# vbronetskyi/nclt-slam-project

Hardware: AMD Instinct MI355X
Metric: relocalization frames/sec @640x480, 10k-landmark DB; Hamming-match HBM GB/s (higher is better)
Workload: dtype u8; 1 GPU; 640x480 BGR frames, 10000-record landmark DB (640000 descriptors, rows=fixed64), global relocalization tick per frame: ORB(500) + whole-DB mutual Hamming scan + top-25 PnP-RANSAC(200); frames resident in HBM, every frame's 96-byte result record written to pinned host memory by the tick's last kernel; distinct_frames=32, preroll_steps=20, streams=4, records=10000, descriptors=640000, parallelism=frames sharded across ranks, database replicated, no collective

## Files before the change

### nclt-slam-project_amd/csrc/reloc_orb.hip

```cpp
#include <math.h>

#include "../../include/reloc_orb_pattern.h"
#include "reloc_internal.h"
#include "reloc_pixels.h"

static_assert(HARRIS_CHUNK == 1024, "k_harris reads one dword per thread");

__constant__ signed char c_pattern[RELOC_ORB_NTESTS * 4];
__constant__ int c_umax[16] = {15, 15, 15, 15, 14, 14, 14, 13, 13, 12, 11, 10, 9, 8, 6, 3};
__constant__ signed char c_ring_dx[16] = {0, 1, 2, 3, 3, 3, 2, 1, 0, -1, -2, -3, -3, -3, -2, -1};
__constant__ signed char c_ring_dy[16] = {3, 3, 2, 1, 0, -1, -2, -3, -3, -3, -2, -1, 0, 1, 2, 3};

__device__ __forceinline__ int find_level(const int *base, int id)
{
    int l = 0;
#pragma unroll
    for (int k = 1; k < NLEV; ++k) l += id >= base[k];
    return l;
}


struct OrbBatch { OrbFrame f[RELOC_BATCH_MAX]; };

__device__ __forceinline__ void pyr_tab_index(const OrbTable *__restrict__ tab, const PyrTile &T, const int (&tbase)[NLEV + 1], int i,
// ... 248 lines not shown
        const int v = (int)p[c_ring_dy[k] * stride + c_ring_dx[k]] - c;
        bright |= (u32)(v > thr) << k;
        dark |= (u32)(v < -thr) << k;
    }
    auto run9 = [](u32 m) {
        u32 x = m | (m << 16);
        u32 y = x & (x >> 1);
        y &= y >> 2;
        y &= y >> 4;
        y &= x >> 8;
        return (y & 0xFFFFu) != 0;
    };
    return run9(bright) ? 1 : (run9(dark) ? -1 : 0);
}

__device__ int fast_corner_score(const uint8_t *p, int stride, int thr, int sign)
{
    const int c = p[0];
    int v[16];
#pragma unroll
    for (int k = 0; k < 16; ++k) v[k] = sign * ((int)p[c_ring_dy[k] * stride + c_ring_dx[k]] - c);
    int m2[16], m4[16], best = 0;
#pragma unroll
    for (int k = 0; k < 16; ++k) m2[k] = min(v[k], v[(k + 1) & 15]);
#pragma unroll
    for (int k = 0; k < 16; ++k) m4[k] = min(m2[k], m2[(k + 2) & 15]);
#pragma unroll
    for (int k = 0; k < 16; ++k) {
        const int m8 = min(m4[k], m4[(k + 4) & 15]);
        const int m9 = min(m8, v[(k + 8) & 15]);
        best = max(best, m9);
    }
    return best > thr ? best - 1 : 0;
}

__device__ __forceinline__ bool fast_run9(u32 x)
{
    u32 y = x & (x >> 1);
    y &= y >> 2;
    y &= y >> 4;
    y &= x >> 8;
    return (y & 0xFFFFu) != 0;
}

struct FastQuad {
    u32 nb[2], nd[2];
    const u32 (*w)[3];
    __device__ __forceinline__ FastQuad(const u32 (&rows)[7][3], int thr) : w(rows)
    {
        const u32 c = rows[3][1];
        const u32 ce = c & 0x00FF00FFu, co = (c >> 8) & 0x00FF00FFu;
        const u32 t2 = (0x7FFFu - (u32)thr) * 0x00010001u;
        nb[0] = t2 - ce; nb[1] = t2 - co;
        nd[0] = t2 + ce; nd[1] = t2 + co;
    }
    template <int DX, int DY>
    __device__ __forceinline__ void flags(u32 (&tb)[2], u32 (&td)[2]) const
    {
        constexpr int b = 4 + DX, q = b >> 2, o = b & 3;
        constexpr u32 sel_e = (u32)o | 0x0C00u | (u32)(o + 2) << 16 | 0x0C000000u;
        constexpr u32 sel_o = (u32)(o + 1) | 0x0C00u | (u32)(o + 3) << 16 | 0x0C000000u;
        const u32 ve = __builtin_amdgcn_perm(w[DY + 3][q + 1], w[DY + 3][q], sel_e);
        const u32 vo = __builtin_amdgcn_perm(w[DY + 3][q + 1], w[DY + 3][q], sel_o);
        tb[0] = ve + nb[0]; tb[1] = vo + nb[1];
        td[0] = nd[0] - ve; td[1] = nd[1] - vo;
    }
    template <int K>
    __device__ __forceinline__ void ring(u32 (&tb)[2], u32 (&td)[2]) const
    {
        constexpr int dx[16] = {0, 1, 2, 3, 3, 3, 2, 1, 0, -1, -2, -3, -3, -3, -2, -1};
        constexpr int dy[16] = {3, 3, 2, 1, 0, -1, -2, -3, -3, -3, -2, -1, 0, 1, 2, 3};
        flags<dx[K], dy[K]>(tb, td);
    }
    __device__ __forceinline__ bool candidate() const
    {
        u32 b0[2], d0[2], b4[2], d4[2], b8[2], d8[2], b12[2], d12[2];
        ring<0>(b0, d0); ring<4>(b4, d4); ring<8>(b8, d8); ring<12>(b12, d12);
        u32 any = 0;
#pragma unroll
        for (int j = 0; j < 2; ++j) {
            any |= (b0[j] & b4[j]) | (b8[j] & b12[j]) | ((b0[j] | b4[j]) & (b8[j] | b12[j]));
            any |= (d0[j] & d4[j]) | (d8[j] & d12[j]) | ((d0[j] | d4[j]) & (d8[j] | d12[j]));
        }
        return (any & 0x80008000u) != 0;
    }
    template <int K>
    __device__ __forceinline__ void shift_in(u32 (&mb)[2], u32 (&md)[2]) const
    {
        u32 tb[2], td[2];
        ring<K>(tb, td);
#pragma unroll
        for (int j = 0; j < 2; ++j) {
            mb[j] = (tb[j] & 0x80008000u) | ((mb[j] >> 1) & 0x7FFF7FFFu);
            md[j] = (td[j] & 0x80008000u) | ((md[j] >> 1) & 0x7FFF7FFFu);
        }
        if constexpr (K < 15) shift_in<K + 1>(mb, md);
    }
    __device__ __forceinline__ void masks(u32 (&mb)[2], u32 (&md)[2]) const
    {
        mb[0] = mb[1] = md[0] = md[1] = 0;
        shift_in<0>(mb, md);
    }
};

constexpr int FT_P = FT / 4 + 3;
static_assert(FT == 32, "fast_nms_tile maps 256 lanes to 32 rows x 8 dwords");
template <bool MASKED, int THR>
__device__ __forceinline__ void fast_nms_tile(const OrbTable *__restrict__ tab, const uint8_t *__restrict__ pyr,
                                              uint8_t *__restrict__ nms, int32_t *__restrict__ hist, int bid,
                                              const uint8_t *__restrict__ mask)
{
    __shared__ u32 s_img4[(FT + 8) * FT_P];
    __shared__ u32 s_sc4[(FT + 2) * (FT + 4) / 4];
    __shared__ unsigned short s_corner[(FT + 2) * (FT + 2)];
    __shared__ int s_nc;
    __shared__ int s_hist[256];
    const uint8_t *const s_img = reinterpret_cast<const uint8_t *>(s_img4);
    uint8_t *const s_sc = reinterpret_cast<uint8_t *>(s_sc4);
    const int l = find_level(tab->fast_tile_base, bid);
    const OrbLevel L = tab->lev[l];
    const int tile = bid - tab->fast_tile_base[l];
    const int tx = L.stride / FT;
    const int x0 = (tile % tx) * FT, y0 = (tile / tx) * FT;
    const int tid = threadIdx.x;
    const int e = RELOC_ORB_EDGE;
    const int thr = THR ? THR : tab->fast_thr;
    uint8_t *out = nms + L.off;
    const bool live = L.quota > 0 && x0 + FT > e && x0 < L.w - e && y0 + FT > e && y0 < L.h - e;
    if (!live) {
        const int y = y0 + tid / 8, x = x0 + (tid % 8) * 4;
        if (y < L.h) *reinterpret_cast<u32 *>(out + (size_t)y * L.stride + x) = 0;
        return;
    }
    s_hist[tid] = 0;
    const uint8_t *src = pyr + L.off;
    const int IS = 4 * FT_P;
    {
        const int r16 = tid >> 4, c16 = tid & 15;
        u32 v[3];
#pragma unroll
        for (int t = 0; t < 3; ++t) {
            const int ry = 16 * t + r16;
            if (c16 < FT / 4 + 2 && ry < FT + 8) {
                const int gy = min(max(y0 + ry - 4, 0), L.h - 1);
                v[t] = halo_dword<false>(src + (size_t)gy * L.stride, x0 - 4 + 4 * c16, L.w);
            }
        }
#pragma unroll
        for (int t = 0; t < 3; ++t) {
            const int ry = 16 * t + r16;
            if (c16 < FT / 4 + 2 && ry < FT + 8) s_img4[ry * FT_P + c16] = v[t];
        }
    }
    for (int i = tid; i < (FT + 2) * (FT + 4) / 4; i += 256) s_sc4[i] = 0;
    if (tid == 0) s_nc = 0;
    __syncthreads();
    const int SS = FT + 4;
    {
        const int ry = 1 + (tid >> 3), g = tid & 7, rx = 1 + 4 * g;
        u32 w[7][3];
#pragma unroll
        for (int r = 0; r < 7; ++r)
#pragma unroll
            for (int q = 0; q < 3; ++q) w[r][q] = s_img4[(ry + r) * FT_P + g + q];
        const FastQuad Q(w, thr);
        if (__any(Q.candidate())) {
            u32 mb[2], md[2];
            Q.masks(mb, md);
            const int gy = y0 + ry - 1;
            const bool row_in = gy >= 3 && gy < L.h - 3;
#pragma unroll
            for (int k = 0; k < 4; ++k) {
                const u32 sel = (k & 2) ? 0x03020302u : 0x01000100u;
                const bool br = fast_run9(__builtin_amdgcn_perm(mb[k & 1], mb[k & 1], sel));
                const bool dk = fast_run9(__builtin_amdgcn_perm(md[k & 1], md[k & 1], sel));
                const int gx = x0 + rx - 1 + k;
                if ((br || dk) && row_in && gx >= 3 && gx < L.w - 3)
                    s_corner[atomicAdd(&s_nc, 1)] = (unsigned short)((ry << 6) | (rx + k) | (br ? 0 : 0x8000));
            }
        }
    }
    {
        const int i = tid;
        const int ry = i < FT + 2 ? 0 : (i < 2 * (FT + 2) ? FT + 1 : (i < 3 * FT + 4 ? i - (2 * FT + 3) : i - (3 * FT + 3)));
        const int rx = i < FT + 2 ? i : (i < 2 * (FT + 2) ? i - (FT + 2) : (i < 3 * FT + 4 ? 0 : FT + 1));
        const int gy = y0 + ry - 1, gx = x0 + rx - 1;
        int pol = 0;
        bool cand = false;
        const uint8_t *pc = s_img + (ry + 3) * IS + (rx + 3);
        const bool inside = i < 4 * FT + 4 && gx >= 3 && gx < L.w - 3 && gy >= 3 && gy < L.h - 3;
        if (inside) {
            const int c = pc[0];
            const int v0 = (int)pc[3 * IS] - c, v4 = (int)pc[3] - c, v8 = (int)pc[-3 * IS] - c, v12 = (int)pc[-3] - c;
            const int nb = (v0 > thr) + (v4 > thr) + (v8 > thr) + (v12 > thr);
            const int nd = (v0 < -thr) + (v4 < -thr) + (v8 < -thr) + (v12 < -thr);
            cand = nb >= 2 || nd >= 2;
        }
        if (tid < 3 * 64 && __any(cand)) {
            if (cand) pol = fast_is_corner(pc, IS, thr);
        }
        if (pol) s_corner[atomicAdd(&s_nc, 1)] = (unsigned short)((ry << 6) | rx | (pol < 0 ? 0x8000 : 0));
    }
    __syncthreads();
    for (int i = tid; i < s_nc; i += 256) {
        const int e16 = s_corner[i], ry = (e16 >> 6) & 63, rx = e16 & 63;
        s_sc[ry * SS + rx] = (uint8_t)fast_corner_score(s_img + (ry + 3) * IS + (rx + 3), IS, thr, (e16 & 0x8000) ? -1 : 1);
    }
    __syncthreads();
    {
        const int ry = tid / 8, rx4 = (tid % 8) * 4;
        u32 word = 0;
        u32 keep = 0;
        if constexpr (MASKED)
            if (y0 + ry < L.h) keep = *reinterpret_cast<const u32 *>(mask + L.off + (size_t)(y0 + ry) * L.stride + x0 + rx4);
#pragma unroll
        for (int k = 0; k < 4; ++k) {
            const int gx = x0 + rx4 + k, gy = y0 + ry;
            const uint8_t *s = s_sc + (ry + 1) * SS + (rx4 + k + 1);
            const int c = (!MASKED || ((keep >> (8 * k)) & 0xFF)) ? s[0] : 0;
            if (c && gx >= e && gx < L.w - e && gy >= e && gy < L.h - e && c > s[-1] && c > s[1] && c > s[-SS - 1] &&
                c > s[-SS] && c > s[-SS + 1] && c > s[SS - 1] && c > s[SS] && c > s[SS + 1]) {
                word |= (u32)c << (8 * k);
                atomicAdd(&s_hist[c], 1);
            }
        }
        const int gy = y0 + ry;
        if (gy < L.h) *reinterpret_cast<u32 *>(out + (size_t)gy * L.stride + x0 + rx4) = word;
    }
    __syncthreads();
    if (s_hist[tid]) atomicAdd(&hist[l * 256 + tid], s_hist[tid]);
}

template <bool MASKED, int THR>
__global__ __launch_bounds__(256) void k_fast_blur(const OrbTable *__restrict__ tab, const uint8_t *__restrict__ pyr,
                                                   uint8_t *__restrict__ nms, int32_t *__restrict__ hist,
                                                   uint8_t *__restrict__ blur, int n_fast, const uint8_t *__restrict__ mask)
{
    RELOC_SMALL_KERNEL_PRIO();
    if ((int)blockIdx.x < n_fast) fast_nms_tile<MASKED, THR>(tab, pyr, nms, hist, (int)blockIdx.x, mask);
    else blur7_tile(tab, pyr, blur, (int)blockIdx.x - n_fast);
}
template <bool MASKED, int THR>
__global__ __launch_bounds__(256) void k_fast_blur_batch(OrbBatch b, int n_fast)
{
    RELOC_SMALL_KERNEL_PRIO();
    const OrbFrame &F = b.f[blockIdx.y];
    if ((int)blockIdx.x < n_fast) fast_nms_tile<MASKED, THR>(F.tab, F.pyr, F.nms, F.hist, (int)blockIdx.x, F.mask);
    else blur7_tile(F.tab, F.pyr, F.blur, (int)blockIdx.x - n_fast);
}

__global__ __launch_bounds__(256) void k_mask_level(const OrbTable *__restrict__ tab, const int32_t *__restrict__ rz,
                                                    uint8_t *__restrict__ mp, int l)
{
    const OrbLevel S = tab->lev[l - 1], D = tab->lev[l];
    const int x4 = 4 * (int)(blockIdx.x * 256 + threadIdx.x), y = (int)blockIdx.y;
    if (x4 >= D.stride || y >= D.h) return;
    const int32_t *xo = rz + tab->rz_off[l][0], *xc = rz + tab->rz_off[l][1];
    const int sy0 = rz[tab->rz_off[l][2] + y], sy1 = sy0 + 1 < S.h ? sy0 + 1 : S.h - 1;
    const u32 b = (u32)rz[tab->rz_off[l][3] + y], one = 1u << RELOC_RESIZE_COEF_BITS;
    const uint8_t *r0 = mp + S.off + (size_t)sy0 * S.stride, *r1 = mp + S.off + (size_t)sy1 * S.stride;
    u32 out = 0;
#pragma unroll
    for (int k = 0; k < 4; ++k) {
        if (x4 + k < D.w) {
            const int k0 = xo[x4 + k], k1 = k0 + 1 < S.w ? k0 + 1 : S.w - 1;
            const u32 a = (u32)xc[x4 + k];
            const u32 h0 = (u32)r0[k0] * (one - a) + (u32)r0[k1] * a;
            const u32 h1 = (u32)r1[k0] * (one - a) + (u32)r1[k1] * a;
            const u32 v = (h0 * (one - b) + h1 * b + (1u << 15)) >> 16;
            if (v > RELOC_ORB_MASK_THRESH) out |= v << (8 * k);
        }
    }
    *reinterpret_cast<u32 *>(mp + D.off + (size_t)y * D.stride + x4) = out;
}

__device__ int stage1_cut_wave(const int32_t *__restrict__ hist_l, int n_keep, int lane, int thr)
{
    const int4 h = *reinterpret_cast<const int4 *>(hist_l + 4 * lane);
    const int mine = h.x + h.y + h.z + h.w;
    int incl = mine;
#pragma unroll
    for (int d = 1; d < 64; d <<= 1) {
        const int v = __shfl_down(incl, d);
        if (lane + d < 64) incl += v;
    }
    const int above = incl - mine;
    const int c3 = h.w + above, c2 = h.z + c3, c1 = h.y + c2, c0 = h.x + c1;
    const int total = __builtin_amdgcn_readlane(c0, 0);
    int cut0 = thr;
    if (total > n_keep) {
        const int s = c3 >= n_keep ? 3 : (c2 >= n_keep ? 2 : (c1 >= n_keep ? 1 : (c0 >= n_keep ? 0 : -1)));
        cut0 = (int)wave_max_u32(s < 0 ? 0u : (unsigned)(4 * lane + s + 1)) - 1;
    }
    unsigned best = 0;
    const int cs[4] = {c0, c1, c2, c3};
#pragma unroll
    for (int k = 3; k >= 0; --k) {
        const int s = 4 * lane + k;
        if (s >= cut0 && (cs[k] <= RELOC_ORB_STAGE1_CAP || s == 255)) best = (unsigned)(256 - s);
    }
    return 256 - (int)wave_max_u32(best);
}

__device__ __forceinline__ void harris_terms(const uint8_t *p, int step, int lane, int &a, int &b, int &c)
{
    a = b = c = 0;
    if (lane < 49) {
        const int dy = lane / 7 - 3, dx = lane % 7 - 3;
        const uint8_t *q = p + dy * step + dx;
        const int ix = (q[1] - q[-1]) * 2 + (q[-step + 1] - q[-step - 1]) + (q[step + 1] - q[step - 1]);
        const int iy = (q[step] - q[-step]) * 2 + (q[step - 1] - q[-step - 1]) + (q[step + 1] - q[-step + 1]);
        a = ix * ix; b = iy * iy; c = ix * iy;
    }
}

__device__ __forceinline__ float harris_finish(int a, int b, int c)
{
    a = wave_sum_i32(a);
    b = wave_sum_i32(b);
    c = wave_sum_i32(c);
    const float scale = __fdiv_rn(1.f, (float)((1 << 2) * RELOC_HARRIS_BLOCK) * 255.f);
    const float s2 = __fmul_rn(scale, scale), s3 = __fmul_rn(s2, scale), s4 = __fmul_rn(s3, scale);
    const float fa = (float)a, fb = (float)b, fc = (float)c;
    const float t1 = __fmul_rn(fa, fb), t2 = __fmul_rn(fc, fc), t3 = __fadd_rn(fa, fb);
    const float t4 = __fmul_rn(RELOC_HARRIS_K, t3), t5 = __fmul_rn(t4, t3);
    const float t6 = __fsub_rn(t1, t2), t7 = __fsub_rn(t6, t5);
    return __fmul_rn(t7, s4);
}

enum { ORB_MODE_DEFAULT = 0, ORB_MODE_HARRIS = 1, ORB_MODE_FAST = 2 };
template <int MODE>
__device__ __forceinline__ void harris_body(const OrbTable *__restrict__ tab, const uint8_t *__restrict__ pyr,
                                                const uint8_t *__restrict__ nms, const int32_t *__restrict__ hist,
                                                int32_t *__restrict__ cand_cnt, u32 *__restrict__ cand_key,
                                                float *__restrict__ cand_resp, int32_t *__restrict__ dbg_cut)
{
    __shared__ int s_cut;
    __shared__ int s_n, s_base;
    __shared__ u32 s_list[HARRIS_CHUNK];
    const int thr = MODE == ORB_MODE_DEFAULT ? RELOC_FAST_THRESHOLD : tab->fast_thr;
    const int l = find_level(tab->flat_base, blockIdx.x);
    const OrbLevel L = tab->lev[l];
    if (L.quota <= 0 || L.w <= 2 * RELOC_ORB_EDGE || L.h <= 2 * RELOC_ORB_EDGE) return;
    const int64_t idx0 = ((int64_t)(blockIdx.x - tab->flat_base[l]) * 256 + threadIdx.x) * (HARRIS_CHUNK / 256);
    const int64_t total = (int64_t)L.stride * L.h;
    u32 v = 0;
    if (idx0 < total) v = *reinterpret_cast<const u32 *>(nms + L.off + idx0);
    const bool any = v != 0;
    if (threadIdx.x == 0) s_n = 0;
    if (!__syncthreads_or(any)) return;
    if (threadIdx.x < 64) {
        const int c = stage1_cut_wave(hist + l * 256, MODE == ORB_MODE_FAST ? L.quota : 2 * L.quota, threadIdx.x, thr);
        if (threadIdx.x == 0) {
            s_cut = c;
            if (dbg_cut) dbg_cut[l] = c;
        }
    }
    __syncthreads();
    const int cut = s_cut;
    if constexpr (MODE == ORB_MODE_FAST) {
        if (any) {
#pragma unroll
            for (int k = 0; k < HARRIS_CHUNK / 256; ++k) {
                const int sc = (v >> (8 * k)) & 0xFF;
                if (sc && sc >= cut) {
                    const int64_t idx = idx0 + k;
                    const int y = (int)(idx / L.stride), x = (int)(idx % L.stride);
                    const int pos = atomicAdd(&cand_cnt[l], 1);
                    if (pos < RELOC_ORB_STAGE1_CAP) {
                        cand_key[(size_t)l * RELOC_ORB_STAGE1_CAP + pos] = ((u32)y << 16) | (u32)x;
                        cand_resp[(size_t)l * RELOC_ORB_STAGE1_CAP + pos] = (float)sc;
                    }
                }
            }
        }
        return;
    }
    if (any) {
#pragma unroll
        for (int k = 0; k < HARRIS_CHUNK / 256; ++k) {
            const int sc = (v >> (8 * k)) & 0xFF;
            if (sc && sc >= cut) {
                const int64_t idx = idx0 + k;
                const int y = (int)(idx / L.stride), x = (int)(idx % L.stride);
                s_list[atomicAdd(&s_n, 1)] = ((u32)y << 16) | (u32)x;
            }
        }
    }
    __syncthreads();
    const int n = s_n;
    const int lane = threadIdx.x & 63, wave = threadIdx.x >> 6;
    const uint8_t *img = pyr + L.off;
    int base_ret = 0;
    if (threadIdx.x == 0 && n > 0) base_ret = atomicAdd(&cand_cnt[l], n);
    auto terms = [&](u32 key, int &a, int &b, int &c) {
        harris_terms(img + (size_t)(key >> 16) * L.stride + (key & 0xFFFF), L.stride, lane, a, b, c);
    };
    int i = wave * 2;
    const bool first = i < n;
    u32 k0 = 0, k1 = 0;
    int a0 = 0, b0 = 0, c0 = 0, a1 = 0, b1 = 0, c1 = 0;
    float h0 = 0.f, h1 = 0.f;
    if (first) {
        k0 = s_list[i]; k1 = s_list[i + 1 < n ? i + 1 : i];
        terms(k0, a0, b0, c0);
        terms(k1, a1, b1, c1);
    }
    if (threadIdx.x == 0) s_base = base_ret;
    if (first) { h0 = harris_finish(a0, b0, c0); h1 = harris_finish(a1, b1, c1); }
    __syncthreads();
    const int base = s_base;
    auto put = [&](int at, u32 key, float r) {
        const int pos = base + at;
        if (pos < RELOC_ORB_STAGE1_CAP) {
            cand_key[(size_t)l * RELOC_ORB_STAGE1_CAP + pos] = key;
            cand_resp[(size_t)l * RELOC_ORB_STAGE1_CAP + pos] = r;
        }
    };
    if (first && lane == 0) {
        put(i, k0, h0);
        if (i + 1 < n) put(i + 1, k1, h1);
    }
    for (i += 8; i < n; i += 8) {
        k0 = s_list[i]; k1 = s_list[i + 1 < n ? i + 1 : i];
        terms(k0, a0, b0, c0);
        terms(k1, a1, b1, c1);
        h0 = harris_finish(a0, b0, c0);
        h1 = harris_finish(a1, b1, c1);
        if (lane == 0) {
            put(i, k0, h0);
            if (i + 1 < n) put(i + 1, k1, h1);
        }
    }
}
template <int MODE>
__global__ __launch_bounds__(256) void k_harris(const OrbTable *__restrict__ tab, const uint8_t *__restrict__ pyr,
                                                const uint8_t *__restrict__ nms, const int32_t *__restrict__ hist,
                                                int32_t *__restrict__ cand_cnt, u32 *__restrict__ cand_key,
                                                float *__restrict__ cand_resp, int32_t *__restrict__ dbg_cut)
{
    RELOC_SMALL_KERNEL_PRIO();
    harris_body<MODE>(tab, pyr, nms, hist, cand_cnt, cand_key, cand_resp, dbg_cut);
}
template <int MODE>
__global__ __launch_bounds__(256) void k_harris_batch(OrbBatch b)
{
    RELOC_SMALL_KERNEL_PRIO();
    const OrbFrame &F = b.f[blockIdx.y];
    harris_body<MODE>(F.tab, F.pyr, F.nms, F.hist, F.cand_cnt, F.cand_key, F.cand_resp, F.dbg_cut);
}

__device__ __forceinline__ void select_body(const OrbTable *__restrict__ tab, const int32_t *__restrict__ cand_cnt,
                                                 const u32 *__restrict__ cand_key, const float *__restrict__ cand_resp,
                                                 int32_t *__restrict__ kp_cnt, u32 *__restrict__ kp_key,
                                                 float *__restrict__ kp_resp)
{
    __shared__ u32 s_key[RELOC_ORB_STAGE1_CAP];
    __shared__ float s_resp[RELOC_ORB_STAGE1_CAP];
    __shared__ u32 s_kidx[RELOC_ORB_STAGE1_CAP];
    __shared__ int s_nk;
    const int l = blockIdx.x;
    const int quota = tab->lev[l].quota;
    const int M = min(cand_cnt[l], RELOC_ORB_STAGE1_CAP);
    const int tid = threadIdx.x;
    if (tid == 0) s_nk = 0;
    for (int i = tid; i < M; i += 1024) {
        s_key[i] = cand_key[(size_t)l * RELOC_ORB_STAGE1_CAP + i];
        s_resp[i] = cand_resp[(size_t)l * RELOC_ORB_STAGE1_CAP + i];
    }
    __syncthreads();
    for (int i = tid; i < M; i += 1024) {
        const float r = s_resp[i];
        int greater = 0;
        for (int j = 0; j < M; ++j) greater += s_resp[j] > r;
        if (greater < quota) s_kidx[atomicAdd(&s_nk, 1)] = (u32)i;
    }
    __syncthreads();
    const int K = s_nk;
    for (int i = tid; i < K; i += 1024) {
        const u32 src = s_kidx[i];
        const u32 key = s_key[src];
        int pos = 0;
        for (int j = 0; j < K; ++j) pos += s_key[s_kidx[j]] < key;
        kp_key[(size_t)l * RELOC_ORB_STAGE1_CAP + pos] = key;
        kp_resp[(size_t)l * RELOC_ORB_STAGE1_CAP + pos] = s_resp[src];
    }
    if (tid == 0) kp_cnt[l] = K;
}
__global__ __launch_bounds__(1024) void k_select(const OrbTable *__restrict__ tab, const int32_t *__restrict__ cand_cnt,
                                                 const u32 *__restrict__ cand_key, const float *__restrict__ cand_resp,
                                                 int32_t *__restrict__ kp_cnt, u32 *__restrict__ kp_key,
                                                 float *__restrict__ kp_resp)
{
    RELOC_SMALL_KERNEL_PRIO();
    select_body(tab, cand_cnt, cand_key, cand_resp, kp_cnt, kp_key, kp_resp);
}
__global__ __launch_bounds__(1024) void k_select_batch(OrbBatch b)
{
    RELOC_SMALL_KERNEL_PRIO();
    const OrbFrame &F = b.f[blockIdx.y];
    select_body(F.tab, F.cand_cnt, F.cand_key, F.cand_resp, F.kp_cnt, F.kp_key, F.kp_resp);
}

__device__ float fast_atan2_deg(float y, float x)
{
    const float ax = fabsf(x), ay = fabsf(y);
    float a;
    if (ax >= ay) {
        const float c = __fdiv_rn(ay, __fadd_rn(ax, RELOC_ATAN2_EPS));
        const float c2 = __fmul_rn(c, c);
        float t = __fadd_rn(__fmul_rn(RELOC_ATAN2_P7, c2), RELOC_ATAN2_P5);
        t = __fadd_rn(__fmul_rn(t, c2), RELOC_ATAN2_P3);
        t = __fadd_rn(__fmul_rn(t, c2), RELOC_ATAN2_P1);
        a = __fmul_rn(t, c);
    } else {
        const float c = __fdiv_rn(ax, __fadd_rn(ay, RELOC_ATAN2_EPS));
        const float c2 = __fmul_rn(c, c);
        float t = __fadd_rn(__fmul_rn(RELOC_ATAN2_P7, c2), RELOC_ATAN2_P5);
        t = __fadd_rn(__fmul_rn(t, c2), RELOC_ATAN2_P3);
        t = __fadd_rn(__fmul_rn(t, c2), RELOC_ATAN2_P1);
        t = __fmul_rn(t, c);
        a = __fsub_rn(90.f, t);
    }
    if (x < 0) a = __fsub_rn(180.f, a);
    if (y < 0) a = __fsub_rn(360.f, a);
    return a;
}

__device__ void sincos_spec(double th, float *s_out, float *c_out)
{
    const double PIO2_HI = 1.57079632679489655800e+00;
    const double PIO2_LO = 6.12323399573676603587e-17;
    const double TWO_OVER_PI = 6.36619772367581382433e-01;
    const double kd = floor(__dadd_rn(__dmul_rn(th, TWO_OVER_PI), 0.5));
    const int k = (int)kd;
    double r = __dsub_rn(th, __dmul_rn(kd, PIO2_HI));
    r = __dsub_rn(r, __dmul_rn(kd, PIO2_LO));
    const double r2 = __dmul_rn(r, r);
    const double S[8] = {-1.0 / 6.0, 1.0 / 120.0, -1.0 / 5040.0, 1.0 / 362880.0, -1.0 / 39916800.0,
                         1.0 / 6227020800.0, -1.0 / 1307674368000.0, 1.0 / 355687428096000.0};
    const double C[8] = {-1.0 / 2.0, 1.0 / 24.0, -1.0 / 720.0, 1.0 / 40320.0, -1.0 / 3628800.0,
                         1.0 / 479001600.0, -1.0 / 87178291200.0, 1.0 / 20922789888000.0};
    double ps = S[7], pc = C[7];
#pragma unroll
    for (int i = 6; i >= 0; --i) {
        ps = __dadd_rn(__dmul_rn(ps, r2), S[i]);
        pc = __dadd_rn(__dmul_rn(pc, r2), C[i]);
    }
    ps = __dmul_rn(__dadd_rn(__dmul_rn(ps, r2), 1.0), r);
    pc = __dadd_rn(__dmul_rn(pc, r2), 1.0);
    double sn, cs;
    switch (k & 3) {
    case 0: sn = ps; cs = pc; break;
    case 1: sn = pc; cs = -ps; break;
    case 2: sn = -ps; cs = -pc; break;
    default: sn = -pc; cs = ps; break;
    }
    *s_out = (float)sn;
    *c_out = (float)cs;
}

__device__ __forceinline__ void describe_body(const OrbTable *__restrict__ tab, const uint8_t *__restrict__ pyr,
                                                  const uint8_t *__restrict__ blur, const int32_t *__restrict__ kp_cnt,
                                                  const u32 *__restrict__ kp_key, const float *__restrict__ kp_resp,
                                                  int max_feat, float *__restrict__ f_xy, float *__restrict__ f_size,
                                                  float *__restrict__ f_angle, float *__restrict__ f_resp,
                                                  int32_t *__restrict__ f_oct, uint8_t *__restrict__ f_desc,
                                                  int32_t *__restrict__ f_count)
{
    const int lane = threadIdx.x & 63;
    const int g = blockIdx.x * 4 + (threadIdx.x >> 6);
    int base[NLEV + 1];
    base[0] = 0;
#pragma unroll
    for (int l = 0; l < NLEV; ++l) base[l + 1] = base[l] + kp_cnt[l];
    const int total = base[NLEV];
    if (g == 0 && lane == 0) *f_count = min(total, max_feat);
    if (g >= total || g >= max_feat) return;
    int l = 0;
#pragma unroll
    for (int k = 1; k < NLEV; ++k) l += g >= base[k];
    const OrbLevel L = tab->lev[l];
    const int i = g - base[l];
    const u32 key = kp_key[(size_t)l * RELOC_ORB_STAGE1_CAP + i];
    const int x = key & 0xFFFF, y = key >> 16;
    const uint8_t *center = pyr + L.off + (size_t)y * L.stride + x;
    int m10 = 0, m01 = 0;
    {
        const int u = (lane & 31) - 15;
        const int half = lane >> 5;
        for (int vv = half; vv <= 30; vv += 2) {
            const int v = vv - 15;
            const int av = v < 0 ? -v : v;
            if (u <= 15 && (u < 0 ? -u : u) <= c_umax[av]) {
                const int I = center[v * L.stride + u];
                m10 += u * I;
                m01 += v * I;
            }
        }
        m10 = wave_sum_i32(m10);
        m01 = wave_sum_i32(m01);
    }
    const float angle = fast_atan2_deg((float)m01, (float)m10);
    float sn, cs;
    sincos_spec((double)__fmul_rn(angle, RELOC_DEG2RAD_F), &sn, &cs);
    const uint8_t *bc = blur + L.off + (size_t)y * L.stride + x;
    unsigned long long bits[4];
#pragma unroll
    for (int it = 0; it < 4; ++it) {
        const signed char *t = c_pattern + 4 * (64 * it + lane);
        int val[2];
#pragma unroll
        for (int e = 0; e < 2; ++e) {
            const float px = (float)t[2 * e], py = (float)t[2 * e + 1];
            const float rx = __fsub_rn(__fmul_rn(px, cs), __fmul_rn(py, sn));
            const float ry = __fadd_rn(__fmul_rn(px, sn), __fmul_rn(py, cs));
            const int ix = (int)rintf(rx), iy = (int)rintf(ry);
            val[e] = bc[iy * L.stride + ix];
        }
        bits[it] = __ballot(val[0] < val[1]);
    }
    if (lane < 4) {
        const unsigned long long b = lane == 0 ? bits[0] : lane == 1 ? bits[1] : lane == 2 ? bits[2] : bits[3];
        reinterpret_cast<unsigned long long *>(f_desc + (size_t)g * 32)[lane] = b;
    }
    if (lane == 0) {
        f_xy[2 * g] = __fmul_rn((float)x, L.scale);
        f_xy[2 * g + 1] = __fmul_rn((float)y, L.scale);
        f_size[g] = __fmul_rn((float)RELOC_ORB_PATCH, L.scale);
        f_angle[g] = angle;
        f_resp[g] = kp_resp[(size_t)l * RELOC_ORB_STAGE1_CAP + i];
        f_oct[g] = l;
    }
}
__global__ __launch_bounds__(256) void k_describe(const OrbTable *__restrict__ tab, const uint8_t *__restrict__ pyr,
                                                  const uint8_t *__restrict__ blur, const int32_t *__restrict__ kp_cnt,
                                                  const u32 *__restrict__ kp_key, const float *__restrict__ kp_resp,
                                                  int max_feat, float *__restrict__ f_xy, float *__restrict__ f_size,
                                                  float *__restrict__ f_angle, float *__restrict__ f_resp,
                                                  int32_t *__restrict__ f_oct, uint8_t *__restrict__ f_desc,
                                                  int32_t *__restrict__ f_count)
{
    RELOC_SMALL_KERNEL_PRIO();
    describe_body(tab, pyr, blur, kp_cnt, kp_key, kp_resp, max_feat, f_xy, f_size, f_angle, f_resp, f_oct, f_desc, f_count);
}
__global__ __launch_bounds__(256) void k_describe_batch(OrbBatch b, int max_feat)
{
    RELOC_SMALL_KERNEL_PRIO();
    const OrbFrame &F = b.f[blockIdx.y];
    describe_body(F.tab, F.pyr, F.blur, F.kp_cnt, F.kp_key, F.kp_resp, max_feat, F.f_xy, F.f_size, F.f_angle, F.f_resp, F.f_oct, F.f_desc,
                  F.f_count);
}

int orb_alloc(reloc_ctx *ctx)
{
    OrbState &o = ctx->orb;
    OrbFrame &b = o.buf;
    const int64_t mf = ctx->max_feat, s1 = (int64_t)NLEV * RELOC_ORB_STAGE1_CAP;
    o.caps = orb_caps(ctx->max_w, ctx->max_h);
    int rc = 0;
    for (uint8_t **p : {&b.pyr, &b.blur, &b.nms}) rc |= ctx_dev_alloc(ctx, p, o.caps.pyr_bytes);
    rc |= ctx_dev_alloc(ctx, &b.tab, 1);
    rc |= ctx_dev_alloc(ctx, &b.rz, o.caps.rz_entries);
    rc |= ctx_dev_alloc(ctx, &b.tiles, o.caps.tiles);
    rc |= ctx_dev_alloc(ctx, &b.hist, NLEV * 256);
    for (int32_t **p : {&b.cand_cnt, &b.kp_cnt, &b.dbg_cut}) rc |= ctx_dev_alloc(ctx, p, NLEV);
    for (uint32_t **p : {&b.cand_key, &b.kp_key}) rc |= ctx_dev_alloc(ctx, p, s1);
    for (float **p : {&b.cand_resp, &b.kp_resp}) rc |= ctx_dev_alloc(ctx, p, s1);
    rc |= ctx_dev_alloc(ctx, &b.f_xy, mf * 2);
    for (float **p : {&b.f_size, &b.f_angle, &b.f_resp}) rc |= ctx_dev_alloc(ctx, p, mf);
    rc |= ctx_dev_alloc(ctx, &b.f_oct, mf);
    rc |= ctx_dev_alloc(ctx, &b.f_desc, mf * 32);
    rc |= ctx_dev_alloc(ctx, &b.f_count, 1);
    return rc;
}

static int orb_grow(reloc_ctx *ctx, const OrbParams &prm)
{
    OrbState &o = ctx->orb;
    const OrbCaps want = orb_caps(ctx->max_w, ctx->max_h, prm);
    if (want.pyr_bytes <= o.caps.pyr_bytes) return RELOC_OK;
    HIP_TRY(hipStreamSynchronize(ctx->stream));
    auto swap_block = [ctx](uint8_t **p, int64_t bytes, int64_t keep) -> int {
        void *q = nullptr;
        HIP_TRY(hipMalloc(&q, (size_t)bytes));
        if (keep > 0) HIP_TRY(hipMemcpy(q, *p, (size_t)keep, hipMemcpyDeviceToDevice));
        for (void *&b : ctx->dev_blocks)
            if (b == (void *)*p) b = q;
        HIP_TRY(hipFree(*p));
        *p = (uint8_t *)q;
        return RELOC_OK;
    };
    for (uint8_t **p : {&o.buf.pyr, &o.buf.blur, &o.buf.nms})
        if (int rc = swap_block(p, want.pyr_bytes, 0)) return rc;
    OrbMaskStage &m = o.mask;
    if (m.pyr) {
        const int64_t level0 = m.on() ? (int64_t)((m.w + 63) / 64 * 64) * m.h : 0;
        if (int rc = swap_block(&m.pyr, 2 * want.pyr_bytes, level0)) return rc;
        m.call = m.pyr + want.pyr_bytes;
        m.built = false;
        m.last = nullptr;
    }
    o.caps.pyr_bytes = want.pyr_bytes;
    o.w = o.h = o.nfeat = 0;
    return RELOC_OK;
}

static bool g_pattern_uploaded[64] = {};

int orb_prepare(reloc_ctx *ctx, int w, int h, int nfeatures, const OrbParams &prm)
{
    OrbState &o = ctx->orb;
    if (w > ctx->max_w || h > ctx->max_h) {
        reloc_set_error("frame %dx%d exceeds the ctx capacity %dx%d", w, h, ctx->max_w, ctx->max_h);
        return RELOC_E_CAPACITY;
    }
    if (o.w == w && o.h == h && o.nfeat == nfeatures && o.plan_prm.same(prm)) return RELOC_OK;
    if (!g_pattern_uploaded[ctx->device & 63]) {
        HIP_TRY(hipMemcpyToSymbol(HIP_SYMBOL(c_pattern), RELOC_ORB_PATTERN, sizeof(RELOC_ORB_PATTERN)));
        g_pattern_uploaded[ctx->device & 63] = true;
    }
    const OrbPlan plan = orb_plan(w, h, nfeatures, o.caps, prm);
    if (plan.rc) { reloc_set_error("%s", plan.err); return plan.rc; }
    o.w = o.h = o.nfeat = 0;
    const hipError_t e0 = hipMemcpyAsync(const_cast<PyrTile *>(o.buf.tiles), plan.tiles.data(), sizeof(PyrTile) * plan.tiles.size(),
                                         hipMemcpyHostToDevice, ctx->stream);
    const hipError_t e1 = hipMemcpyAsync(const_cast<int32_t *>(o.buf.rz), plan.rz.data(), sizeof(int32_t) * plan.rz.size(),
                                         hipMemcpyHostToDevice, ctx->stream);
    const hipError_t e2 = hipMemcpyAsync(const_cast<OrbTable *>(o.buf.tab), &plan.tab, sizeof(OrbTable), hipMemcpyHostToDevice, ctx->stream);
    const hipError_t e3 = hipStreamSynchronize(ctx->stream);
    HIP_TRY(e0); HIP_TRY(e1); HIP_TRY(e2); HIP_TRY(e3);
    memcpy(&o.tab, &plan.tab, sizeof(OrbTable));
    o.lds = plan.lds; o.lds_bytes = plan.lds_bytes; o.ntiles = (int)plan.tiles.size();
    o.w = w; o.h = h; o.nfeat = nfeatures; o.plan_prm = prm;
    return RELOC_OK;
// ... 269 lines not shown
```

Before: 7644 frames/s.

## Compute Harris response with 8-lane groups per keypoint using row-wise separable Sobel

Restructures the Harris scoring so each wave processes 8 keypoints at once, with each 8-lane group handling one candidate and each lane computing one row of the 7x7 window via dword loads and separable Sobel sums. The full 64-lane wave reduction becomes a 3-step DPP reduction within 8 lanes. Candidate filtering is precomputed into a bitmask and the key is derived with a single 32-bit divide instead of per-candidate 64-bit div/mod. This aims to cut wasted lanes (previously 15 of 64 idle) and reduction cost, at the cost of unaligned dword loads and more per-lane arithmetic.

```diff
diff --git a/nclt-slam-project_amd/csrc/reloc_orb.hip b/nclt-slam-project_amd/csrc/reloc_orb.hip
--- a/nclt-slam-project_amd/csrc/reloc_orb.hip
+++ b/nclt-slam-project_amd/csrc/reloc_orb.hip
@@ -574,23 +574,47 @@
     return 256 - (int)wave_max_u32(best);
 }
 
-__device__ __forceinline__ void harris_terms(const uint8_t *p, int step, int lane, int &a, int &b, int &c)
-{
+__device__ __forceinline__ u32 harris_load4(const uint8_t *p)
+{
+    u32 v;
+    __builtin_memcpy(&v, p, 4);
+    return v;
+}
+__device__ __forceinline__ void harris_row_terms(const uint8_t *p, int step, int r, int &a, int &b, int &c)
+{
+    const uint8_t *q = p + (r - 3) * step - 4;
+    int cs[9], d[9];
+#pragma unroll
+    for (int w = 0; w < 3; ++w) {
+        const u32 t = harris_load4(q - step + 4 * w), m = harris_load4(q + 4 * w), u = harris_load4(q + step + 4 * w);
+#pragma unroll
+        for (int k = 4 * w; k < 4 * w + 4 && k < 9; ++k) {
+            const int sh = 8 * (k & 3), tk = (t >> sh) & 0xFF, mk = (m >> sh) & 0xFF, uk = (u >> sh) & 0xFF;
+            cs[k] = tk + 2 * mk + uk;
+            d[k] = uk - tk;
+        }
+    }
     a = b = c = 0;
-    if (lane < 49) {
-        const int dy = lane / 7 - 3, dx = lane % 7 - 3;
-        const uint8_t *q = p + dy * step + dx;
-        const int ix = (q[1] - q[-1]) * 2 + (q[-step + 1] - q[-step - 1]) + (q[step + 1] - q[step - 1]);
-        const int iy = (q[step] - q[-step]) * 2 + (q[step - 1] - q[-step - 1]) + (q[step + 1] - q[-step + 1]);
-        a = ix * ix; b = iy * iy; c = ix * iy;
-    }
+#pragma unroll
+    for (int j = 0; j < 7; ++j) {
+        const int ix = cs[j + 2] - cs[j], iy = d[j] + 2 * d[j + 1] + d[j + 2];
+        a += ix * ix; b += iy * iy; c += ix * iy;
+    }
+}
+
+__device__ __forceinline__ int group8_sum_i32(int x)
+{
+    x += __builtin_amdgcn_update_dpp(0, x, 0xB1, 0xF, 0xF, false);
+    x += __builtin_amdgcn_update_dpp(0, x, 0x4E, 0xF, 0xF, false);
+    x += __builtin_amdgcn_update_dpp(0, x, 0x141, 0xF, 0xF, false);
+    return x;
 }
 
 __device__ __forceinline__ float harris_finish(int a, int b, int c)
 {
-    a = wave_sum_i32(a);
-    b = wave_sum_i32(b);
-    c = wave_sum_i32(c);
+    a = group8_sum_i32(a);
+    b = group8_sum_i32(b);
+    c = group8_sum_i32(c);
     const float scale = __fdiv_rn(1.f, (float)((1 << 2) * RELOC_HARRIS_BLOCK) * 255.f);
     const float s2 = __fmul_rn(scale, scale), s3 = __fmul_rn(s2, scale), s4 = __fmul_rn(s3, scale);
     const float fa = (float)a, fb = (float)b, fc = (float)c;
@@ -598,6 +622,12 @@
     const float t4 = __fmul_rn(RELOC_HARRIS_K, t3), t5 = __fmul_rn(t4, t3);
     const float t6 = __fsub_rn(t1, t2), t7 = __fsub_rn(t6, t5);
     return __fmul_rn(t7, s4);
+}
+
+__device__ __forceinline__ u32 harris_key0(int64_t idx0, int stride)
+{
+    const u32 i = (u32)idx0, y = i / (u32)stride;
+    return y << 16 | (i - y * (u32)stride);
 }
 
 enum { ORB_MODE_DEFAULT = 0, ORB_MODE_HARRIS = 1, ORB_MODE_FAST = 2 };
@@ -630,34 +660,33 @@
     }
     __syncthreads();
     const int cut = s_cut;
+    u32 keep = 0;
+#pragma unroll
+    for (int k = 0; k < HARRIS_CHUNK / 256; ++k) {
+        const int sc = (v >> (8 * k)) & 0xFF;
+        keep |= (u32)(sc && sc >= cut) << k;
+    }
     if constexpr (MODE == ORB_MODE_FAST) {
-        if (any) {
+        if (keep) {
+            const u32 key0 = harris_key0(idx0, L.stride);
 #pragma unroll
             for (int k = 0; k < HARRIS_CHUNK / 256; ++k) {
-                const int sc = (v >> (8 * k)) & 0xFF;
-                if (sc && sc >= cut) {
-                    const int64_t idx = idx0 + k;
-                    const int y = (int)(idx / L.stride), x = (int)(idx % L.stride);
+                if (keep >> k & 1) {
                     const int pos = atomicAdd(&cand_cnt[l], 1);
                     if (pos < RELOC_ORB_STAGE1_CAP) {
-                        cand_key[(size_t)l * RELOC_ORB_STAGE1_CAP + pos] = ((u32)y << 16) | (u32)x;
-                        cand_resp[(size_t)l * RELOC_ORB_STAGE1_CAP + pos] = (float)sc;
+                        cand_key[(size_t)l * RELOC_ORB_STAGE1_CAP + pos] = key0 + k;
+                        cand_resp[(size_t)l * RELOC_ORB_STAGE1_CAP + pos] = (float)((v >> (8 * k)) & 0xFF);
                     }
                 }
             }
         }
         return;
     }
-    if (any) {
-#pragma unroll
-        for (int k = 0; k < HARRIS_CHUNK / 256; ++k) {
-            const int sc = (v >> (8 * k)) & 0xFF;
-            if (sc && sc >= cut) {
-                const int64_t idx = idx0 + k;
-                const int y = (int)(idx / L.stride), x = (int)(idx % L.stride);
-                s_list[atomicAdd(&s_n, 1)] = ((u32)y << 16) | (u32)x;
-            }
-        }
+    if (keep) {
+        const u32 key0 = harris_key0(idx0, L.stride);
+#pragma unroll
+        for (int k = 0; k < HARRIS_CHUNK / 256; ++k)
+            if (keep >> k & 1) s_list[atomicAdd(&s_n, 1)] = key0 + k;
     }
     __syncthreads();
     const int n = s_n;
@@ -665,44 +694,34 @@
     const uint8_t *img = pyr + L.off;
     int base_ret = 0;
     if (threadIdx.x == 0 && n > 0) base_ret = atomicAdd(&cand_cnt[l], n);
-    auto terms = [&](u32 key, int &a, int &b, int &c) {
-        harris_terms(img + (size_t)(key >> 16) * L.stride + (key & 0xFFFF), L.stride, lane, a, b, c);
+    const int grp = lane >> 3, r = lane & 7;
+    u32 key = 0;
+    auto response = [&](int at) {
+        int a = 0, b = 0, c = 0;
+        if (at < n && r < RELOC_HARRIS_BLOCK) {
+            key = s_list[at];
+            harris_row_terms(img + (size_t)(key >> 16) * L.stride + (key & 0xFFFF), L.stride, r, a, b, c);
+        }
+        return harris_finish(a, b, c);
     };
-    int i = wave * 2;
+    int i = wave * 8;
     const bool first = i < n;
-    u32 k0 = 0, k1 = 0;
-    int a0 = 0, b0 = 0, c0 = 0, a1 = 0, b1 = 0, c1 = 0;
-    float h0 = 0.f, h1 = 0.f;
-    if (first) {
-        k0 = s_list[i]; k1 = s_list[i + 1 < n ? i + 1 : i];
-        terms(k0, a0, b0, c0);
-        terms(k1, a1, b1, c1);
-    }
+    float resp = 0.f;
+    if (first) resp = response(i + grp);
     if (threadIdx.x == 0) s_base = base_ret;
-    if (first) { h0 = harris_finish(a0, b0, c0); h1 = harris_finish(a1, b1, c1); }
     __syncthreads();
     const int base = s_base;
-    auto put = [&](int at, u32 key, float r) {
+    auto put = [&](int at, float v) {
         const int pos = base + at;
-        if (pos < RELOC_ORB_STAGE1_CAP) {
+        if (at < n && r == 0 && pos < RELOC_ORB_STAGE1_CAP) {
             cand_key[(size_t)l * RELOC_ORB_STAGE1_CAP + pos] = key;
-            cand_resp[(size_t)l * RELOC_ORB_STAGE1_CAP + pos] = r;
+            cand_resp[(size_t)l * RELOC_ORB_STAGE1_CAP + pos] = v;
         }
     };
-    if (first && lane == 0) {
-        put(i, k0, h0);
-        if (i + 1 < n) put(i + 1, k1, h1);
-    }
-    for (i += 8; i < n; i += 8) {
-        k0 = s_list[i]; k1 = s_list[i + 1 < n ? i + 1 : i];
-        terms(k0, a0, b0, c0);
-        terms(k1, a1, b1, c1);
-        h0 = harris_finish(a0, b0, c0);
-        h1 = harris_finish(a1, b1, c1);
-        if (lane == 0) {
-            put(i, k0, h0);
-            if (i + 1 < n) put(i + 1, k1, h1);
-        }
+    if (first) put(i + grp, resp);
+    for (i += 32; i < n; i += 32) {
+        resp = response(i + grp);
+        put(i + grp, resp);
     }
 }
 template <int MODE>
```

Measured after the change: 7648 frames/s (median of 2 runs). Within noise of the previous version (+0.1%).
